# t-neumann/versalignLib

Hardware: AMD Instinct MI355X
Metric: GCUPS (giga DP cell updates/sec) SW affine-gap, 150x500 bp (higher is better)
Workload: dtype int16; 1 GPU; 1048576 pairs/GPU, 150 bp x 500 bp, SW affine-gap int16 score (open -5, extend -1), inputs resident in HBM; pairs_per_gpu=1048576, read_length=150, ref_length=500, kernel_geometry=16x10

## Files before the change

### versalignlib_amd/csrc/cell_rules.h

```cpp
#pragma once

#include <algorithm>
#include <cstdlib>
#include <stdexcept>
#include <string>

#include "cell_constants.h"

namespace valign {

struct RuleInputs {
    Scoring sc;
    int R = 0, F = 0;
    bool sse_policy = false;
    bool no_sym = false, no_tag = false, no_f16 = false, no_prof_key = false;
    bool no_max3 = false;
    bool no_tilt = false;
};

inline long long nw_tilt_span(const Scoring &sc, int rows, int F) {
    const long long per_row = -(long long)(sc.affine ? sc.ext_ref : sc.gap_ref);
    const long long per_col = -(long long)(sc.affine ? sc.ext_read : sc.gap_read);
    return per_row * (rows + 1) + per_col * (F + 1);
}

inline bool half_float_exact(const Scoring &sc, int alg, int R, int F, int rows) {
    const long long top = (long long)std::min(R, F) * std::max({sc.match, sc.mismatch, 0});
    long long slack = std::max({std::abs(sc.match), std::abs(sc.mismatch), std::abs(sc.open_read),
                                std::abs(sc.ext_read), std::abs(sc.open_ref), std::abs(sc.ext_ref)});
    if (alg == kAlgSW) return top + 2 * slack <= 2048 && slack <= 1024;
    if (!sc.affine) slack = std::max<long long>(slack, std::max(std::abs(sc.gap_read), std::abs(sc.gap_ref)));
    const long long span = nw_tilt_span(sc, rows, F);
    const long long centre = (top + span) / 2;
    return span < 30000 && (top + span - centre) + 3 * slack <= 2048 && centre + 3 * slack <= 2048 && slack <= 512;
}

inline bool half_float_unit_exact(const Scoring &sc, int R, int F) {
    const long long top = (long long)std::min(R, F) * std::max({sc.match, sc.mismatch, 0});
    const long long slack = std::max({std::abs(sc.match), std::abs(sc.mismatch), std::abs(sc.gap_read), std::abs(sc.gap_ref)});
    return top + 2 * slack < 1024 && slack < 512;
// ... 89 lines not shown
    if (sc.open_ref > 0 || sc.ext_ref > 0) return false;
    const long long B = sym_affine_bias(sc);
    const long long hi = (long long)std::min(R, F) * std::max({sc.match, sc.mismatch, 0}) + 1;
    return B - kMax3WindowLow <= 1024 && B + hi <= kMax3WindowHigh;
}
inline const char *ran_sym_affine_name(bool max3) { return max3 ? "max3" : "sources"; }

inline int sym_affine_tilt_bias(const Scoring &sc) {
    const int o = -sc.open_ref, x = -sc.ext_ref, m = std::max({0, -sc.mismatch, -sc.match});
    return kMax3WindowLow + std::max(o - x, m);
}
inline long long sym_affine_tilt_top_index(int R, int F, int rows, int K) {
    const int lead = rows > R ? (rows - R) / K : 0;
    return (long long)rows + F - lead;
}
inline bool sym_affine_tilt_ok(const RuleInputs &in, int R, int F, int rows, int K) {
    if (in.no_tilt || K > kTiltMaxK || !sym_affine_max3_ok(in, R, F)) return false;
    const Scoring &sc = in.sc;
    const long long B = sym_affine_tilt_bias(sc);
    const long long hi = (long long)std::min(R, F) * std::max({sc.match, sc.mismatch, 0}) + 1;
    return B + (long long)-sc.ext_ref * sym_affine_tilt_top_index(R, F, rows, K) + hi <= kMax3WindowHigh;
}
inline const char *ran_sym_affine_frame_name(bool tilted) { return tilted ? "tilted" : "plain"; }

struct FillChoice {
    int kernel = 0;
    bool affine_tagged = false, tagged = false;
};
inline FillChoice fill_choice(const RuleInputs &in, int alg, int G, int K) {
    const Scoring &sc = in.sc;
    FillChoice c;
    const int rows = G * K;
    c.affine_tagged = sc.affine && !in.sse_policy && !in.no_tag && affine_tagged_range_ok(in, alg, rows, K);
    c.tagged = !sc.affine && !in.no_tag && tagged_range_ok(in, alg, rows);
    const bool lane_key = c.tagged && alg == kAlgSW && lane_key_ok(in, K);
    const bool prof_key = lane_key && prof_key_ok(in, K);
    const bool affine_sym = sc.affine && sc.open_read == sc.open_ref && sc.ext_read == sc.ext_ref && !in.no_sym;
    if (prof_key) c.kernel = kFillTagProfKey;
    else if (c.tagged) c.kernel = in.sse_policy ? (lane_key ? kFillSseTagKey : kFillSseTag) : (lane_key ? kFillTagKey : kFillTag);
    else if (in.sse_policy) c.kernel = kFillSse;
    else if (sc.affine) c.kernel = c.affine_tagged ? (affine_sym ? kFillAffineTagSym : kFillAffineTag) : (affine_sym ? kFillAffineSym : kFillAffine);
    else c.kernel = (sc.gap_read == sc.gap_ref && !in.no_sym) ? kFillLinearSym : kFillLinear;
    return c;
}

constexpr int placed_key_bits(int K) { return K <= 4 ? 2 : (K <= 8 ? 3 : 4); }
// ... 255 lines not shown
```

### versalignlib_amd/csrc/dp_kernels.hip.h

```cpp
#pragma once

#include <hip/hip_runtime.h>
#include <stdint.h>

#include <type_traits>
#include <utility>

#include "base_classes.h"
#include "cell_constants.h"

namespace valign {

typedef short s16x2 __attribute__((ext_vector_type(2)));
typedef _Float16 f16x2 __attribute__((ext_vector_type(2)));
typedef unsigned short u16x2 __attribute__((ext_vector_type(2)));

constexpr int kWave = 64;
constexpr int kWaveLanes = 64;
constexpr int kCodePad = 72;
constexpr short kNegInf = -16384;

constexpr int kMaxScoreGroups = 16;
constexpr int kOneSweep = 0x7FFFFFFF;

// ... 369 lines not shown
    }
    if (live) {
        for (int idx = lane; idx < geo::kPairStride / 4; idx += kWave) {
            const unsigned lo = (unsigned short)(zero_score + row_key_step * (15 - (2 * idx) % K) + ((2 * idx) % K == 0 ? row0_score : 0));
            const unsigned hi = (unsigned short)(zero_score + row_key_step * (15 - (2 * idx + 1) % K) + ((2 * idx + 1) % K == 0 ? row0_score : 0));
            reinterpret_cast<unsigned *>(prof + geo::kZeroSlab * geo::kPairStride)[idx] = lo | (hi << 16);
        }
    }
    __syncthreads();
#pragma unroll
    for (int d = kWave / 2; d >= 1; d >>= 1) {
        const int other = __shfl_xor(cols_used, d, kWave);
        cols_used = other > cols_used ? other : cols_used;
    }
    w.cols_used = __builtin_amdgcn_readfirstlane(cols_used);
    w.prof = prof;
    w.refc = refc + 2 * kCodePad;
    w.first_bad = first_bad;
    w.pair0 = pair0;
    w.last = last;
    return live;
}

template <int K>
__device__ __forceinline__ void lds_load_lane(unsigned addr, unsigned (&v)[K / 2]) {
    constexpr int N = K / 2;
    if constexpr ((K * 2) % 16 == 0) {
#pragma unroll
        for (int i = 0; i < N / 4; ++i) {
            const u32x4 x = *(lds_cu32x4 *)(addr + 16 * i);
            v[4 * i] = x.x; v[4 * i + 1] = x.y; v[4 * i + 2] = x.z; v[4 * i + 3] = x.w;
        }
    } else if constexpr ((K * 2) % 8 == 0) {
#pragma unroll
        for (int i = 0; i < N / 2; ++i) {
            const u32x2 x = *(lds_cu32x2 *)(addr + 8 * i);
            v[2 * i] = x.x; v[2 * i + 1] = x.y;
        }
    } else {
#pragma unroll
        for (int i = 0; i < N; ++i) v[i] = *(lds_cu32 *)(addr + 4 * i);
    }
}

template <int K>
__device__ __forceinline__ void merge_profile(const unsigned (&va)[K / 2], const unsigned (&vb)[K / 2], s16x2 (&S)[K]) {
// ... 62 lines not shown
    int fold = tilt_row + tilt_col;
    short s_row0 = 0;
    if constexpr (SOURCES && K <= kTiltMaxK) {
        if (args.sym_max3_bias > 0 && (args.sym_max3_bias >> 16) != 0) {
            fold = -2 * (int)args.ext_ref;
            s_row0 = (short)((int)args.ext_ref - (int)args.open_ref);
        }
    }
    const int centre = (HALF && TILT) ? nw_frame_centre(args.R, F_batch, G * K, args.match, args.mismatch, tilt_row, tilt_col) : 0;
    const int rcentre = (HALF && TILT) ? nw_frame_centre(args.R, F_batch, G * K, args.match, args.mismatch, 0, 0) : 0;
    const float unit = LINF16_SW ? 1.0f / 1024.0f : 1.0f;
    auto cell = [](int v) __attribute__((always_inline)) {
        return HALF ? pk(__builtin_bit_cast(short, (_Float16)v)) : pk((short)v);
    };
    auto cell_add = [](s16x2 a, s16x2 b) __attribute__((always_inline)) {
        return HALF ? __builtin_bit_cast(s16x2, __builtin_bit_cast(f16x2, a) + __builtin_bit_cast(f16x2, b)) : a + b;
    };
    auto cell_sub = [](s16x2 a, s16x2 b) __attribute__((always_inline)) {
        return HALF ? __builtin_bit_cast(s16x2, __builtin_bit_cast(f16x2, a) - __builtin_bit_cast(f16x2, b)) : a - b;
    };
    const short s_match = HALF ? __builtin_bit_cast(short, (_Float16)(((int)args.match + fold) * unit)) : (short)(args.match + fold);
    const short s_mismatch = HALF ? __builtin_bit_cast(short, (_Float16)(((int)args.mismatch + fold) * unit)) : (short)(args.mismatch + fold);
    const short s_zero = HALF ? __builtin_bit_cast(short, (_Float16)fold) : (short)fold;
    if (!wave_setup<G, K, false>(reads, refs, n_pairs, args.R, F_batch, args.prof_area, args.refc_stride,
                                 args.wave_lds, s_match, s_mismatch, w, false, block, s_zero, kOneSweep, 0, s_row0))
        return;
    const long long pair0 = w.pair0;
    const int F = (ALG == kAlgSW) ? w.cols_used : F_batch;

    const unsigned lmask = l == 0 ? 0u : 0xFFFFFFFFu;
    const unsigned lane_base = lds_offset(w.prof) + l * geo::kLaneBytes;
    const int lead = (ALG == kAlgSW && G * K > args.R) ? (G * K - args.R) / K : 0;
    unsigned code_addr = lds_offset(w.refc) + grp * args.refc_stride - 2 * (l - lead);

    s16x2 g_read, g_ref, o_read, e_read, o_ref, e_ref;
    if (ALG == kAlgSW) {
        g_read = pk((short)-args.gap_read);   g_ref = pk((short)-args.gap_ref);
        o_read = pk((short)-args.open_read);  e_read = pk((short)-args.ext_read);
        o_ref = pk((short)-args.open_ref);    e_ref = pk((short)-args.ext_ref);
    } else {
        g_read = g_ref = e_read = e_ref = pk(0);
        o_read = pk((short)(args.open_read - args.ext_read));
        o_ref = pk((short)(args.open_ref - args.ext_ref));
    }
    const s16x2 border_f = pk(ALG == kAlgNW ? (F16 ? (short)0xFC00 : kNegInf) : (short)0);
    const _Float16 open_h = (_Float16)(int)(TILT ? args.open_ref - args.ext_ref : args.open_ref), ext_h = (_Float16)(int)args.ext_ref;
    const _Float16 open_rd = (_Float16)(int)(TILT ? args.open_read - args.ext_read : args.open_read), ext_rd = (_Float16)(int)args.ext_read;
    const f16x2 o_half = f16x2{open_h, open_h}, e_half = f16x2{ext_h, ext_h}, zero_half = f16x2{(_Float16)0, (_Float16)0};
// ... 5 lines not shown
        Hl[q] = cell(tilt_row * (l * K + q) - centre);
        El[q] = border_f;
        HOl[q] = (ALG == kAlgSW) ? pk(0) : (F16 ? cell_add(Hl[q], pk(__builtin_bit_cast(short, open_h))) : Hl[q] + o_ref);
    }
    s16x2 up0 = pk(0), h_last = Hl[K - 1], f_last = border_f, best = pk(0);
    s16x2 fup_keep = border_f;
    s16x2 row_best = cell(-rcentre);
    int j = -l;
    s16x2 top_row = pk(0), top_step = pk(0), row_tilt = pk(0);
    const s16x2 col_step = cell(tilt_col);
    if (TILT) {
        if (l == 0) {
            top_row = cell(-tilt_row + tilt_col - centre);
            top_step = col_step;
            up0 = cell(-tilt_row - centre);
        }
        row_tilt = cell(tilt_row * (G * K - 1) + tilt_col * (1 - l) - centre + rcentre);
    }

    constexpr bool PIPE = true;
    unsigned pa[K / 2], pb[K / 2];
    s16x2 S0[K], S1[K];
    unsigned ca_next = 0, cb_next = 0;
    if (PIPE) {
        const unsigned ca = *(lds_cu8 *)(code_addr), cb = *(lds_cu8 *)(code_addr + 1);
        lds_load_lane<K>(lane_base + ca * geo::kPairStride, pa);
        lds_load_lane<K>(lane_base + cb * geo::kPairStride, pb);
        ca_next = *(lds_cu8 *)(code_addr + 2);
        cb_next = *(lds_cu8 *)(code_addr + 3);
    }

    lds_cu8 *code_ptr = (lds_cu8 *)code_addr;

    auto step = [&](auto masked_tag, auto track_tag, s16x2 (&S)[K], s16x2 (&Snext)[K]) __attribute__((always_inline)) {
        constexpr bool MASKED = decltype(masked_tag)::value;
        constexpr int TRACK = decltype(track_tag)::value;
        const s16x2 diag0 = up0;
        if (G == 16) {
            up0 = as_pk((unsigned)__builtin_amdgcn_update_dpp(0, (int)as_u32(h_last), 0x111, 0xF, 0xF, true));
        } else {
            up0 = as_pk(from_prev_lane(as_u32(h_last)) & lmask);
        }
        if (TILT) up0 = as_pk(as_u32(up0) | as_u32(top_row));
        s16x2 fup0 = border_f;
        if (AFFINE && !SOURCES) {
            if (G == 16 && ALG == kAlgSW) {
                fup0 = as_pk((unsigned)__builtin_amdgcn_update_dpp(0, (int)as_u32(f_last), 0x111, 0xF, 0xF, true));
// ... 210 lines not shown
        if constexpr (SOURCES) {
            biased = args.sym_max3_bias > 0;
            const bool tilted = K <= kTiltMaxK && biased && (args.sym_max3_bias >> 16) != 0;
            if constexpr (K <= kTiltMaxK) if (tilted) {
                const int B = args.sym_max3_bias & 0xFFFF, xi = -(int)args.ext_ref;
                const int oxi = -(int)args.open_ref - xi;
                const s16x2 ox_c = pk((short)oxi), kx_c = pk((short)(K * xi));
                const int u0 = l * (K - 1);
                s16x2 lead_border = as_pk(as_u32(pk((short)(B + xi - oxi))) & ~lmask);
                const s16x2 lead_step = as_pk(as_u32(pk((short)xi)) & ~lmask);
                const int s0 = K - steps % K;
                s16x2 fl[K], acc[K], dprev[K];
#pragma unroll
                for (int q = 0; q < K; ++q) {
                    Hl[q] = El[q] = pk((short)(B + xi * (u0 + q + 1)));
                    HOl[q] = Hl[q] - ox_c;
                    int c = q - s0;
                    c += c < 0 ? K : 0;
                    fl[q] = acc[q] = pk((short)(B + xi * (u0 + c + 2)));
                    dprev[q] = Hl[q];
                }
                up0 = pk((short)(B + xi * u0 - oxi));
                f_last = HOl[K - 1];
                auto tilted_step = [&](auto slot_tag) __attribute__((always_inline)) {
                    constexpr int SLOT0 = decltype(slot_tag)::value;
                    s16x2 S[K], d[K];
                    const s16x2 diag0 = up0;
                    up0 = group_prev_or<G>(HOl[K - 1], lead_border, lmask);
                    lead_border = lead_border + lead_step;
                    merge_profile<K>(pa, pb, S);
                    lds_load_lane<K>(lane_base + ca_next * geo::kPairStride, pa);
                    lds_load_lane<K>(lane_base + cb_next * geo::kPairStride, pb);
                    ca_next = ((volatile lds_cu8 *)code_ptr)[4];
                    cb_next = ((volatile lds_cu8 *)code_ptr)[5];
                    s16x2 e_cur;
                    auto pass1 = [&](int q, s16x2 &e) __attribute__((always_inline)) {
                        d[q] = (q == 0 ? diag0 : Hl[q - 1]) + S[q];
                        e = pk_max3_h(El[q], HOl[q], fl[(q + SLOT0) % K]);
                        El[q] = e;
                    };
                    s16x2 ho = up0;
                    pass1(0, e_cur);
                    s16x2 f = as_pk(group_prev_or_zero<G>(as_u32(f_last), lmask)), h = pk(0);
#pragma unroll
                    for (int q = 0; q < K; ++q) {
                        f = pk_max_h(f, ho);
                        s16x2 e_next = pk(0);
                        if (q + 1 < K) pass1(q + 1, e_next);
                        h = pk_max3_h(d[q], e_cur, f);
                        Hl[q] = h;
                        ho = h - ox_c;
                        HOl[q] = ho;
                        if (!(q & 1)) {
                            s16x2 &a = acc[(q + SLOT0) % K];
                            a = pk_max3_h(a, d[q], dprev[q + 1]);
                        }
                        e_cur = e_next;
                    }
#pragma unroll
                    for (int q = 1; q < K; q += 2) dprev[q] = d[q];
                    f_last = f;
                    acc[SLOT0 % K] = acc[SLOT0 % K] + kx_c;
                    fl[SLOT0 % K] = fl[SLOT0 % K] + kx_c;
                    code_ptr += 2;
                };
                unrolled_steps(std::make_integer_sequence<int, K>{}, [&](auto slot_tag) __attribute__((always_inline)) {
                    if constexpr (decltype(slot_tag)::value > 0) {
                        if (decltype(slot_tag)::value >= s0) tilted_step(slot_tag);
                    }
                });
                for (int trips = steps / K; trips > 0; --trips)
                    unrolled_steps(std::make_integer_sequence<int, K>{}, [&](auto slot_tag) __attribute__((always_inline)) { tilted_step(slot_tag); });
                best = pk(0);
#pragma unroll
                for (int q = 0; q < K; q += 2) acc[q] = pk_max_h(acc[q], dprev[q + 1]);
#pragma unroll
                for (int q = 0; q < K; ++q) best = pk_max(best, acc[q] - fl[q]);
            }
            if (biased && !tilted) {
                const s16x2 bias_c = pk((short)args.sym_max3_bias);
                const s16x2 lead_bias = as_pk(as_u32(bias_c) & ~lmask);
                auto biased_step = [&](s16x2 (&S)[K]) __attribute__((always_inline)) {
                    const s16x2 diag0 = up0;
                    up0 = group_prev_or<G>(h_last, lead_bias, lmask);
                    merge_profile<K>(pa, pb, S);
                    lds_load_lane<K>(lane_base + ca_next * geo::kPairStride, pa);
                    lds_load_lane<K>(lane_base + cb_next * geo::kPairStride, pb);
                    ca_next = code_ptr[4];
                    cb_next = code_ptr[5];
                    s16x2 d_cur, e_cur, d_prev = bias_c;
                    auto pass1 = [&](int q, s16x2 &d, s16x2 &e) __attribute__((always_inline)) {
                        d = (q == 0 ? diag0 : Hl[q - 1]) + S[q];
                        e = pk_max3_h(El[q] - e_read, HOl[q], bias_c);
                        El[q] = e;
                    };
// ... 90 lines not shown
        } else {
            if (pa < n_pairs) scores[pa] = res.x;
            if (pa + 1 < n_pairs) scores[pa + 1] = res.y;
        }
    }
}

struct WaveLds {
    int prof_area, refc_stride, total;
};

template <int G, int K>
inline WaveLds wave_lds(int R, int F) {
    using geo = Geo<G, K>;
    WaveLds w;
    const int raw_refs = ((2 * F + 16 + 15) / 16) * 16;
    w.prof_area = geo::kProfBytes > raw_refs ? geo::kProfBytes : raw_refs;
    w.prof_area = ((w.prof_area + 15) / 16) * 16;
    w.refc_stride = ((2 * (F + 2 * kCodePad) + 15) / 16) * 16;
    w.total = w.prof_area + geo::kGroups * w.refc_stride + ((geo::kPairs * 8 + 15) / 16) * 16;
    return w;
}

}
```

### versalignlib_amd/csrc/engine.hip.h

```cpp
#pragma once

#include <hip/hip_runtime.h>
#include <stdint.h>
#include <stdio.h>
#include <stdlib.h>
#include <string.h>

#include <algorithm>
#include <atomic>
#include <chrono>
#include <condition_variable>
#include <functional>
#include <map>
#include <memory>
#include <mutex>
#include <stdexcept>
#include <string>
#include <thread>
#include <utility>
#include <vector>

#include "align_parts.h"
#include "cell_rules.h"
#include "hip_handles.h"
// ... 92 lines not shown
};
constexpr int kNumGeometries = sizeof(kGeometries) / sizeof(kGeometries[0]);
#define VALIGN_COUNT(G, K) +1
static_assert(kNumGeometries == 0 VALIGN_ALL_PARTS(VALIGN_COUNT, VALIGN_COUNT), "kernel_instances.hip.h lists other geometries than this table");
#undef VALIGN_COUNT

constexpr int kMaxBlockLds = 160 * 1024;
constexpr int kSlots = 4;
constexpr int kDefaultBlockLds = 64 * 1024;

struct LaunchPlan {
    bool long_mode = false;
    const Geometry *geo = nullptr;
    WaveLds lds{};
    int waves_per_block = 4;
    int pairs_per_wave = 0;
};

class DebugSwitches {
public:
    DebugSwitches() {
        const char *env = getenv("VALIGN_HIP_DEBUG");
        if (!env) return;
        static const char *const known[] = {"no_sym", "no_tag", "no_f16", "no_max3", "no_tilt", "no_fused", "no_prof_key", "no_overlap", "no_band_chain",
                                            "force_long", "wide_align", "strip_k", "no_single_strip", "no_direct_out", "ragged_min", "chunk_bytes",
                                            "align_chunk_bytes", "direct_bytes", "scratch_cap_mb", "whole_rows", "short_strips", "cigar_rows_mb", "cigar_lanes",
                                            "span_scratch_bytes", "subopt_scratch_bytes", "span_cigar_mb"};
        std::string s(env);
        for (size_t at = 0; at <= s.size();) {
            const size_t end = std::min(s.find(',', at), s.size());
            const std::string item = s.substr(at, end - at);
            at = end + 1;
            if (item.empty()) continue;
            const size_t eq = item.find('=');
            const std::string name = item.substr(0, eq);
            bool ok = false;
            for (const char *k : known) ok = ok || name == k;
            if (!ok) throw std::runtime_error("VALIGN_HIP_DEBUG: unknown switch '" + name + "'");
            kv_[name] = eq == std::string::npos ? 1 : atoll(item.c_str() + eq + 1);
        }
    }
    bool on(const char *name) const { return kv_.count(name) != 0; }
    long long value(const char *name, long long fallback) const {
        auto it = kv_.find(name);
        return it == kv_.end() ? fallback : it->second;
    }

// ... 99 lines not shown
    void launch_score(const LaunchPlan &plan, int alg, int R, int F, long long n, const uint8_t *d_reads,
                      const uint8_t *d_refs, int16_t *d_scores, hipStream_t stream,
                      const LengthGroup *groups = nullptr, int n_groups = 0);


    void launch_unpack(const uint8_t *d_packed, uint8_t *d_out, long long n, int len, hipStream_t stream);

    LongFacts long_facts(int alg) const {
        return LongFacts{band_width_, band_nw_, score_wide_cells(alg), dbg_.on("short_strips"), dbg_.on("no_single_strip"), no_band_chain_, band_plan_.usable};
    }
    LongScoreMode long_mode(int alg, bool refuse) const { return long_score_mode(rule_inputs(), alg, long_facts(alg), refuse); }

    void score_long_device(int alg, long long n, const uint8_t *d_reads, const uint8_t *d_refs, int16_t *d_scores, hipStream_t stream);
    void sync_band_tables(hipStream_t stream);
    void score_band_device(const LongScoreMode &mode, long long n, const uint8_t *d_reads, const uint8_t *d_refs, int16_t *d_scores, PlacedRec *d_placed,
                           hipStream_t stream);

    const char *score_cell_format(int alg, long long n = 0) const;
    std::string ran_score_cells() const;
    const char *ran_align_fill() const { return ran_align_fill_; }
    static std::string ran_geometry(const Geometry *g) { return g ? std::to_string(g->G) + "x" + std::to_string(g->K) : "none"; }
    std::string ran_kernels() const;

    RuleInputs rule_inputs() const { return RuleInputs{sc_, R_, F_, sse_policy_, no_sym_, no_tag_, no_f16_, no_prof_key_, no_max3_, no_tilt_}; }
    bool score_int16_ok(int alg) const;
    bool score_wide_cells(int alg) const { return score_width_ == 32 || (score_width_ == 0 && !score_int16_ok(alg)); }

    void score_host(int opt, int n, const char *const *reads, const char *const *refs, short *scores,
                    int threads, int16_t *d_dest = nullptr);



    struct WalkChain {
        int region;
        long long chunk_pairs;
        int *min_start;
        uint8_t *packed;
    };
    hipEvent_t trace_done(int region) const { return trace_done_[region].get(); }
    const LaunchPlan &align_plan_for(int alg, FillChoice &choice);
    const LaunchPlan &align_base_plan() const {
        if (plan_.long_mode && align_resident_.geo && !align_resident_.long_mode && R_ <= 1024 && align_resident_.lds.total <= 140 * 1024) {
            const int wpb = align_resident_.waves_per_block;
            const int waves_per_cu = (kMaxBlockLds / std::max(1, align_resident_.lds.total * wpb)) * wpb;
            if (waves_per_cu >= 2 || !sc_.affine) return align_resident_;
        }
        return plan_;
// ... 294 lines not shown
    bool band_nw_ = false;
    bool band_placed_ = false;
    bool placed_wide_ = false;
    bool trace_checkpoints_ = false;
    int score_width_ = 0;
    int ragged_ = 0, force_g_ = 0, force_k_ = 0;
    size_t score_chunk_bytes_ = 48u << 20;
    size_t align_chunk_bytes_ = 128u << 20;
    size_t direct_bytes_ = 768u << 10;
    long long ragged_min_ = 2048;
    std::vector<int> read_caps_, ref_caps_;
    std::vector<unsigned char> read_class_;
    std::vector<unsigned short> ref_class_;
    std::map<std::pair<int, int>, LaunchPlan> class_plans_;
    hipStream_t ragged_dev_stream_ = nullptr;
    HostPacker packer_{R_, F_};
    HostStats host_stats_;
    DebugSwitches dbg_;
    bool no_sym_ = dbg_.on("no_sym");
    bool no_tag_ = dbg_.on("no_tag");
    bool no_f16_ = dbg_.on("no_f16");
    bool no_max3_ = dbg_.on("no_max3");
    bool no_tilt_ = dbg_.on("no_tilt");
    bool no_fused_ = dbg_.on("no_fused");
    bool no_prof_key_ = dbg_.on("no_prof_key");
    bool copy_engines_primed_ = false;
    std::unique_ptr<CopyIssuer> copy_issuer_;
    bool wide_align_ = dbg_.on("wide_align");
    bool whole_rows_ = dbg_.on("whole_rows");
    bool no_direct_out_ = dbg_.on("no_direct_out");
    bool no_overlap_ = dbg_.on("no_overlap");
    int strip_k_ = (int)dbg_.value("strip_k", 0);
    long long scratch_cap_mb_ = dbg_.value("scratch_cap_mb", 0);
    bool chain_regions_busy_[2] = {false, false};
    std::string arch_;
    LaunchPlan plan_, latency_plan_;
    LaunchPlan base_plan_;
    LaunchPlan align_resident_;
    LaunchPlan fallback_plan_;
    long long slot_begin_[kSlots] = {}, slot_pending_[kSlots] = {};
    long long staged_pairs_ = 0, align_staged_pairs_ = 0;
    size_t record_staged_bytes_ = 0;
    bool pack_ = true;
    BandPlan band_plan_;
    int band_tables_width_ = -1;
    int band_blocks_per_cu_ = 0, band_lds_ = 0;
    int long_strip_rows_ = 0;
    static constexpr unsigned kRanF16 = 1, kRanInt16 = 2, kRanInt32 = 4;
    unsigned ran_score_cells_ = 0;
    const char *ran_align_fill_ = "none";
    const Geometry *ran_score_geo_ = nullptr, *ran_align_geo_ = nullptr;
    const Geometry *ran_placed_geo_ = nullptr, *ran_subopt_geo_ = nullptr, *ran_extend_geo_ = nullptr;
    const char *ran_score_sym_affine_ = nullptr;
    const char *ran_score_sym_affine_frame_ = "plain";
    const char *ran_placed_ = "none";
    std::string ran_span_ = "none";
    size_t span_scratch_bytes_ = (size_t)dbg_.value("span_scratch_bytes", 256ll << 20);
    std::string ran_span_cigar_ = "none";
    size_t span_cigar_bytes_ = (size_t)std::max(0ll, dbg_.value("span_cigar_mb", 768)) << 20;
    const char *ran_subopt_ = "none";
    int subopt_ring_cols_ = 0;
    size_t subopt_scratch_bytes_ = (size_t)dbg_.value("subopt_scratch_bytes", 256ll << 20);
    const char *ran_extend_ = "none";
    const char *ran_result_format_ = "rows";
    long long cigar_d2h_bytes_ = 0;
    const CigarSink *cigar_ = nullptr;
    long long cigar_pairs_[2] = {0, 0};
    long long align_ptr_bytes_per_pair_ = 0;
    long long align_ckpt_bytes_per_pair_ = 0;
    int cu_count_ = 0;
    bool no_band_chain_ = dbg_.on("no_band_chain");
    int start_col_[kSlots] = {};

    StreamHandle streams_[kSlots];
    EventHandle slot_done_[kSlots];
    EventHandle in_done_[kSlots], kernels_done_[kSlots];
    StreamHandle trace_stream_;
// ... 43 lines not shown
```

### versalignlib_amd/csrc/engine_core.hip

```cpp
#include "engine.hip.h"

namespace valign {

Engine::Engine(int device, int R, int F, const Scoring &sc, int force_g, int force_k)
    : device_(device), R_(R), F_(F), sc_(sc) {
    if (R < 0 || F < 0) throw std::runtime_error("negative sequence length");
    if ((long long)R + F > 32767)
        throw std::runtime_error("read_length + ref_length exceeds the ABI's 16-bit coordinates");
    validate_scoring();
    int count = 0;
    hip_check(hipGetDeviceCount(&count), "hipGetDeviceCount");
    if (device < 0 || device >= count)
        throw std::runtime_error("HIP device " + std::to_string(device) + " not present (" +
                                 std::to_string(count) + " visible): libHIPKernel.so has no CPU path");
    hip_check(hipSetDevice(device_), "hipSetDevice");
    hipDeviceProp_t prop;
    hip_check(hipGetDeviceProperties(&prop, device_), "hipGetDeviceProperties");
    arch_ = prop.gcnArchName;
    cu_count_ = prop.multiProcessorCount;
    if (arch_.find("gfx950") == std::string::npos)
        throw std::runtime_error("device is " + arch_ + "; this library carries gfx950 code only");
    force_g_ = force_g;
    force_k_ = force_k;
    plan_ = choose_plan(R_, F_, force_g, force_k);
// ... 74 lines not shown
             "\"ran_span_cigar\": \"%s\", \"span_cigar_scratch_bytes\": %lld, "
             "\"ran_subopt\": \"%s\", \"subopt_scratch_bytes\": %lld, \"subopt_ring_cols\": %d, \"ran_extend\": \"%s\", "
             "\"ran_score_geometry\": \"%s\", \"ran_align_geometry\": \"%s\", "
             "\"ran_placed_geometry\": \"%s\", \"ran_subopt_geometry\": \"%s\", \"ran_extend_geometry\": \"%s\"}",
             arch_.c_str(), device_, opt & 0xF, sc_.affine ? 1 : 0, plan_.geo->G, plan_.geo->K,
             plan_.geo->G * plan_.geo->K, plan_.pairs_per_wave, plan_.waves_per_block, plan_.lds.total,
             plan_.lds.total * plan_.waves_per_block, F_ + plan_.geo->G - 1, n > 0 ? (n + ppb - 1) / ppb : 0,
             plan_.long_mode ? 1 : 0, band_width_, ragged_, host_stats_.launches,
             host_stats_.cells_padded > 0 ? host_stats_.cells_swept / host_stats_.cells_padded : 1.0,
             score_cell_format(opt & 0xF, n), host_stats_.direct, host_stats_.packed, host_stats_.direct_out,
             ((opt & 0xF) == kAlgSW || band_nw_) ? band_rows : VALIGN_HIP_BAND_BLOCK_ROWS, ((opt & 0xF) == kAlgSW || band_nw_) ? band_align : VALIGN_HIP_BAND_COL_ALIGN,
             band_blocks_per_cu_, band_lds_, (band_tables_width_ == band_width_ && band_plan_.usable) ? band_plan_.cells : 0ll, long_strip_rows_, host_stats_.d2h_row_bytes / 1e6, host_stats_.full_row_bytes / 1e6, host_stats_.gather_ms, host_stats_.classify_ms, host_stats_.wait_ms,
             host_stats_.drain_ms, ran_score_cells().c_str(), ran_align_fill_, band_alignments(), band_nw(), band_placed(), align_ptr_bytes_per_pair_, trace_checkpoints(),
             align_ckpt_bytes_per_pair_, (long long)d_ptr_.bytes(), ran_result_format_, cigar_d2h_bytes_,
             (long long)(d_cig_rows_[0].bytes() + d_cig_rows_[1].bytes()), ran_placed_, placed_wide(), (long long)(d_placed_rows_.bytes() + d_placed_ends_.bytes()),
             ran_span_.c_str(), span_ref_length(rule_inputs()), (long long)span_[kSlots].bytes(),
             ran_span_cigar_.c_str(), (long long)(span_cigar_[0].bytes() + span_cigar_[1].bytes()),
             ran_subopt_, (long long)subopt_[kSlots].bytes(), subopt_ring_cols_, ran_extend_,
             ran_geometry(ran_score_geo_).c_str(), ran_geometry(ran_align_geo_).c_str(),
             ran_geometry(ran_placed_geo_).c_str(), ran_geometry(ran_subopt_geo_).c_str(), ran_geometry(ran_extend_geo_).c_str());
    std::string out(buf);
    if (ran_score_sym_affine_)
        out.insert(out.size() - 1, std::string(", \"ran_score_sym_affine\": \"") + ran_score_sym_affine_ + "\", \"ran_score_sym_affine_frame\": \"" +
                                       ran_score_sym_affine_frame_ + "\"");
    return out;
}

void Engine::band_block_shape(int &block_rows, int &col_align) const {
    const bool chain = long_mode(kAlgSW, false).chain;
    block_rows = chain ? kBandK : VALIGN_HIP_BAND_BLOCK_ROWS;
    col_align = chain ? VALIGN_HIP_BAND_CHAIN_COL_ALIGN : VALIGN_HIP_BAND_COL_ALIGN;
}

void Engine::validate_scoring() {
    auto fits = [](int v) { return v >= -32768 && v <= 32767; };
    if (!fits(sc_.match) || !fits(sc_.mismatch) || !fits(sc_.gap_read) || !fits(sc_.gap_ref) ||
        !fits(sc_.open_read) || !fits(sc_.ext_read) || !fits(sc_.open_ref) || !fits(sc_.ext_ref))
        throw std::runtime_error("scoring parameter outside int16");
    const bool gaps_ok = sc_.affine ? (sc_.open_read <= 0 && sc_.ext_read <= 0 && sc_.open_ref <= 0 && sc_.ext_ref <= 0)
                                    : (sc_.gap_read <= 0 && sc_.gap_ref <= 0);
    if (!gaps_ok) throw std::runtime_error("positive gap scores are not supported by the HIP kernels");
    if (sc_.affine && (sc_.ext_read < sc_.open_read || sc_.ext_ref < sc_.open_ref))
        throw std::runtime_error("affine gap scores need extend >= open in each direction (an extension dearer "
                                 "than the opening is not an affine model)");
}

LaunchPlan Engine::choose_plan(int R, int F, int force_g, int force_k, bool latency, bool full_only) const {
// ... 166 lines not shown
```

### versalignlib_amd/csrc/engine_score.hip

```cpp
#define VALIGN_TU_SCORE 1
#include "engine.hip.h"

namespace valign {

void Engine::score_device(int opt, long long n, const uint8_t *d_reads, const uint8_t *d_refs,
                  int16_t *d_scores, hipStream_t stream, bool length_sorted) {
    const int alg = opt & 0xF;
    if (alg > 1 || n <= 0) return;
    hip_check(hipSetDevice(device_), "hipSetDevice");
    if (length_sorted) {
        host_stats_ = HostStats{};
        ran_score_cells_ = 0;
        ran_score_geo_ = nullptr;
        ran_score_sym_affine_ = nullptr;
    }
    if (score_width_ == 16 && !score_int16_ok(alg))
        throw std::runtime_error("shape x scoring can leave the int16 range of the DP cells (read_length " +
                                 std::to_string(R_) + ", ref_length " + std::to_string(F_) + ")");
    const bool wide = score_wide_cells(alg);
    if (plan_.long_mode || wide) {
        score_long_device(alg, n, d_reads, d_refs, d_scores, stream);
        return;
    }
    if (length_sorted && ragged_applies(alg) && ragged_fits(n) && n >= 2 * ragged_min_) {
// ... 30 lines not shown
            blocks += (groups[g].pairs + pairs_per_block - 1) / pairs_per_block;
            if (blocks > 0x7FFFFFFFll) throw std::runtime_error("batch too large for one launch");
            a.groups[g].block_end = (unsigned)blocks;
            a.groups[g].F = groups[g].F;
            a.groups[g].n = groups[g].pairs;
            a.groups[g].pair_ofs = groups[g].pair_ofs;
            a.groups[g].read_ofs = (long long)groups[g].read_ofs;
            a.groups[g].ref_ofs = (long long)groups[g].ref_ofs;
        }
    }
    a.prof_area = plan.lds.prof_area;
    a.refc_stride = plan.lds.refc_stride;
    a.wave_lds = plan.lds.total;
    put_scoring(a);
    const int gaps = score_gap_form(rule_inputs(), alg, R, F, plan.geo->G * plan.geo->K);
    const void *fn = plan.geo->kernel[alg][gaps];
    ran_score_cells_ |= gap_form_f16(gaps) ? kRanF16 : kRanInt16;
    ran_score_geo_ = plan.geo;
    if (alg == kAlgSW && gaps == kGapAffineSym) {
        const bool max3 = sym_affine_max3_ok(rule_inputs(), R_, F_);
        a.sym_max3_bias = max3 ? sym_affine_bias(sc_) : 0;
        const bool tilted = sym_affine_tilt_ok(rule_inputs(), R_, F_, plan.geo->G * plan.geo->K, plan.geo->K);
        if (tilted) a.sym_max3_bias = sym_affine_tilt_bias(sc_) | 1 << 16;
        ran_score_sym_affine_ = ran_sym_affine_name(max3);
        ran_score_sym_affine_frame_ = ran_sym_affine_frame_name(tilted);
    }
    const int block_lds = plan.lds.total * plan.waves_per_block;
    if (block_lds > kDefaultBlockLds)
        hip_check(hipFuncSetAttribute(fn, hipFuncAttributeMaxDynamicSharedMemorySize, block_lds),
                  "hipFuncSetAttribute(MaxDynamicSharedMemorySize)");
    if (blocks > 0x7FFFFFFFll) throw std::runtime_error("batch too large for one launch");
    if (blocks == 0) return;
    void *kargs[] = {&a};
    hip_check(hipLaunchKernel(fn, dim3((unsigned)blocks), dim3(plan.waves_per_block * kWave), kargs,
                              (size_t)block_lds, stream),
              "hipLaunchKernel(score_kernel)");
}

void Engine::launch_unpack(const uint8_t *d_packed, uint8_t *d_out, long long n, int len, hipStream_t stream) {
    if (n <= 0 || len <= 0) return;
    UnpackArgs a{d_packed, d_out, n, len};
    void *kargs[] = {&a};
    const bool even = (len & 1) == 0;
    const long long items = even ? (n * (long long)(len / 2) + 7) / 8 : n * (long long)((len + 1) / 2);
    const long long blocks = (items + 255) / 256;
    if (blocks > 0x7FFFFFFFll) throw std::runtime_error("batch too large for one launch");
    hip_check(hipLaunchKernel(even ? (const void *)&unpack_even_kernel : (const void *)&unpack_odd_kernel, dim3((unsigned)blocks),
                              dim3(256), kargs, 0, stream),
              "hipLaunchKernel(unpack_kernel)");
}
// ... 348 lines not shown
```

Baseline: 8964 GCUPS.

## Use per-lane register score tables with byte-select streams in tilted affine SW

Adds a row-table path for the tilted symmetric-affine SW kernel. Each lane builds packed byte tables of substitution scores for its read rows in registers, and the reference is rewritten as per-column perm selectors in LDS. Each DP step then fetches one selector dword and uses v_perm to form the scores, instead of loading profile rows from LDS indexed by reference codes. This lowers LDS traffic per step and shrinks the LDS footprint, but adds register pressure (Ta/Tb arrays), a more complex setup phase and an extra repair variant for non-ACGT columns.

After: 9607 GCUPS (median of 6 runs). 7.2% higher.

```diff
diff --git a/versalignlib_amd/csrc/cell_rules.h b/versalignlib_amd/csrc/cell_rules.h
--- a/versalignlib_amd/csrc/cell_rules.h
+++ b/versalignlib_amd/csrc/cell_rules.h
@@ -16,6 +16,7 @@
     bool no_sym = false, no_tag = false, no_f16 = false, no_prof_key = false;
     bool no_max3 = false;
     bool no_tilt = false;
+    bool no_row_tables = false;
 };
 
 inline long long nw_tilt_span(const Scoring &sc, int rows, int F) {
@@ -151,6 +152,17 @@
     return B + (long long)-sc.ext_ref * sym_affine_tilt_top_index(R, F, rows, K) + hi <= kMax3WindowHigh;
 }
 inline const char *ran_sym_affine_frame_name(bool tilted) { return tilted ? "tilted" : "plain"; }
+
+inline int sym_affine_row_table_low(const Scoring &sc) { return std::min({sc.match, sc.mismatch, 0}) - 2 * sc.ext_ref; }
+inline int sym_affine_row_table_high(const Scoring &sc) {
+    return std::max({sc.match, sc.mismatch, 0}) - 2 * sc.ext_ref + (sc.ext_ref - sc.open_ref);
+}
+inline bool sym_affine_row_tables_ok(const RuleInputs &in, int R, int F, int rows, int K, int lds_profile, int lds_tables) {
+    if (in.no_row_tables || !sym_affine_tilt_ok(in, R, F, rows, K)) return false;
+    if (in.sc.ext_ref - in.sc.open_ref < 0 || F > 60000) return false;
+    return sym_affine_row_table_low(in.sc) >= 0 && sym_affine_row_table_high(in.sc) <= 255 && lds_tables <= lds_profile;
+}
+inline const char *ran_sym_affine_scores_name(bool row_tables) { return row_tables ? "row_tables" : "lds_profile"; }
 
 struct FillChoice {
     int kernel = 0;
diff --git a/versalignlib_amd/csrc/dp_kernels.hip.h b/versalignlib_amd/csrc/dp_kernels.hip.h
--- a/versalignlib_amd/csrc/dp_kernels.hip.h
+++ b/versalignlib_amd/csrc/dp_kernels.hip.h
@@ -415,6 +415,146 @@
     return live;
 }
 
+constexpr int row_table_pad(int G) { return G + 4; }
+constexpr unsigned kSelZero4 = 0x0c0c0c0cu;
+
+template <int G, int K>
+__device__ __forceinline__ bool wave_setup_tables(const uint8_t *reads, const uint8_t *refs, long long n, int R, int F,
+                                                  int refs_area, int sel_stride, int wave_lds, short match, short mismatch,
+                                                  short zero_score, short row0_score, unsigned block, WaveTables &w,
+                                                  unsigned (&Ta)[K], unsigned (&Tb)[K], bool &repair) {
+    using geo = Geo<G, K>;
+    constexpr int kPad = row_table_pad(G);
+    const int lane = threadIdx.x & (kWave - 1);
+    const int wave = threadIdx.x / kWave;
+    const int row0 = R - geo::kRows;
+
+    unsigned char *raw = valign_smem + (size_t)wave * wave_lds;
+    unsigned char *sel = raw + refs_area;
+
+    const int waves = blockDim.x / kWave;
+    const long long pair0 = ((long long)block * waves + wave) * geo::kPairs;
+    const bool live = pair0 < n;
+    long long pair_end = pair0 + geo::kPairs;
+    if (pair_end > n) pair_end = n;
+    const int last = (int)(pair_end - pair0) - 1;
+
+    if (live) {
+        stage_span(raw, refs, pair0 * F, pair_end * F, lane);
+        stage_span(sel, reads, pair0 * R, pair_end * R, lane);
+    }
+    __syncthreads();
+
+    if (live) {
+        auto table = [&](int c, unsigned &lo, unsigned &hi) __attribute__((always_inline)) {
+            unsigned b[8];
+#pragma unroll
+            for (int a = 0; a < 8; ++a) b[a] = (unsigned)(a >= 1 && a <= 4 ? (a == c + 1 ? match : mismatch) : zero_score) & 0xFFu;
+            lo = b[0] | b[1] << 8 | b[2] << 16 | b[3] << 24;
+            hi = b[4] | b[5] << 8 | b[6] << 16 | b[7] << 24;
+        };
+        unsigned t_lo[4], t_hi[4];
+#pragma unroll
+        for (int c = 0; c < 4; ++c) table(c, t_lo[c], t_hi[c]);
+        const unsigned char *raw_rd = sel + (int)((unsigned long long)(reads + pair0 * R) & 15ull);
+        const int grp = lane / G, l = lane % G;
+#pragma unroll
+        for (int half = 0; half < 2; ++half) {
+            int p = 2 * grp + half;
+            p = p > last ? last : p;
+#pragma unroll
+            for (int q0 = 0; q0 < K; q0 += 4) {
+                const int pos = row0 + l * K + q0;
+                const int at = pos < -3 ? -3 : pos;
+                unsigned w4 = lds_dword_at(raw_rd + p * R + at);
+                if (pos < 0) w4 = pos < -3 ? 0u : w4 & (0xFFFFFFFFu << (8 * -pos));
+                const unsigned cls = base_class4(w4);
+                unsigned col[4];
+#pragma unroll
+                for (int c = 0; c < 4; ++c) col[c] = select_bytes8(t_hi[c], t_lo[c], cls);
+                const unsigned lo01 = __builtin_amdgcn_perm(col[1], col[0], 0x05010400u), hi01 = __builtin_amdgcn_perm(col[1], col[0], 0x07030602u);
+                const unsigned lo23 = __builtin_amdgcn_perm(col[3], col[2], 0x05010400u), hi23 = __builtin_amdgcn_perm(col[3], col[2], 0x07030602u);
+                unsigned (&T)[K] = half ? Tb : Ta;
+                T[q0] = __builtin_amdgcn_perm(lo23, lo01, 0x05040100u);
+                T[q0 + 1] = __builtin_amdgcn_perm(lo23, lo01, 0x07060302u);
+                if (q0 + 2 < K) {
+                    T[q0 + 2] = __builtin_amdgcn_perm(hi23, hi01, 0x05040100u);
+                    T[q0 + 3] = __builtin_amdgcn_perm(hi23, hi01, 0x07060302u);
+                }
+            }
+        }
+        const unsigned r4 = ((unsigned)row0_score & 0xFFu) * 0x01010101u;
+        Ta[0] += r4;
+        Tb[0] += r4;
+    }
+    __syncthreads();
+
+    int cols_used = 0;
+    bool before_last = false;
+    unsigned *stream = reinterpret_cast<unsigned *>(sel);
+    const int stride_dw = sel_stride / 4;
+    if (live) {
+        for (int idx = lane; idx < geo::kGroups * 2 * kPad; idx += kWave) {
+            const int g = idx / (2 * kPad), x = idx - g * (2 * kPad);
+            stream[g * stride_dw + (x < kPad ? x : F + x)] = kSelZero4;
+        }
+        const int ref_skew = (int)((unsigned long long)(refs + pair0 * F) & 15ull);
+        typedef unsigned short u16;
+#pragma unroll
+        for (int g = 0; g < geo::kGroups; ++g) {
+            int pa = 2 * g, pb = 2 * g + 1;
+            pa = pa > last ? last : pa;
+            pb = pb > last ? last : pb;
+            const unsigned char *raw_a = raw + ref_skew + pa * F, *raw_b = raw + ref_skew + pb * F;
+            unsigned *out_g = stream + g * stride_dw + kPad;
+            u16x2 ends_a = u16x2{0, 0}, ends_b = u16x2{0, 0};
+            auto note = [](u16x2 &ends, unsigned acgt, int j) __attribute__((always_inline)) {
+                const unsigned none = ~nonzero_bytes(acgt) & 0x80808080u;
+                const u16 end = acgt ? (u16)(j + 4 - (__builtin_clz(acgt) >> 3)) : (u16)0;
+                const u16 first_none = none ? (u16)(0xFFFF - (j + (__builtin_ctz(none) >> 3))) : (u16)0;
+                ends = __builtin_elementwise_max(ends, u16x2{end, first_none});
+            };
+            const int F4 = F & ~3;
+            for (int j = 4 * lane; j < F4; j += 4 * kWave) {
+                const unsigned ca = base_class4(lds_dword_at(raw_a + j)), cb = base_class4(lds_dword_at(raw_b + j));
+                const unsigned sa = select_bytes8(0x0c0c0c03u, 0x0201000cu, ca), sb = select_bytes8(0x0c0c0c07u, 0x0605040cu, cb);
+                uint4 s;
+                s.x = __builtin_amdgcn_perm(sb, sa, 0x0c040c00u) | 0x0c000c00u;
+                s.y = __builtin_amdgcn_perm(sb, sa, 0x0c050c01u) | 0x0c000c00u;
+                s.z = __builtin_amdgcn_perm(sb, sa, 0x0c060c02u) | 0x0c000c00u;
+                s.w = __builtin_amdgcn_perm(sb, sa, 0x0c070c03u) | 0x0c000c00u;
+                *reinterpret_cast<uint4 *>(out_g + j) = s;
+                note(ends_a, sa ^ kSelZero4, j);
+                note(ends_b, sb ^ kSelZero4, j);
+            }
+            for (int j = F4 + lane; j < F; j += kWave) {
+                const int ca = base_class(raw_a[j]), cb = base_class(raw_b[j]);
+                const bool va = ca >= 1 && ca <= 4, vb = cb >= 1 && cb <= 4;
+                out_g[j] = (va ? (unsigned)(ca - 1) : 0x0cu) | (vb ? (unsigned)(cb + 3) : 0x0cu) << 16 | 0x0c000c00u;
+                ends_a = __builtin_elementwise_max(ends_a, u16x2{va ? (u16)(j + 1) : (u16)0, va ? (u16)0 : (u16)(0xFFFF - j)});
+                ends_b = __builtin_elementwise_max(ends_b, u16x2{vb ? (u16)(j + 1) : (u16)0, vb ? (u16)0 : (u16)(0xFFFF - j)});
+            }
+#pragma unroll
+            for (int d = kWave / 2; d >= 1; d >>= 1) {
+                ends_a = __builtin_elementwise_max(ends_a, __builtin_bit_cast(u16x2, __shfl_xor(__builtin_bit_cast(int, ends_a), d, kWave)));
+                ends_b = __builtin_elementwise_max(ends_b, __builtin_bit_cast(u16x2, __shfl_xor(__builtin_bit_cast(int, ends_b), d, kWave)));
+            }
+            before_last |= 0xFFFF - (int)ends_a.y < (int)ends_a.x || 0xFFFF - (int)ends_b.y < (int)ends_b.x;
+            cols_used = (int)ends_a.x > cols_used ? (int)ends_a.x : cols_used;
+            cols_used = (int)ends_b.x > cols_used ? (int)ends_b.x : cols_used;
+        }
+    }
+    __syncthreads();
+    repair = __builtin_amdgcn_readfirstlane((int)before_last) != 0;
+    w.cols_used = __builtin_amdgcn_readfirstlane(cols_used);
+    w.prof = raw;
+    w.refc = reinterpret_cast<unsigned char *>(stream + kPad);
+    w.first_bad = nullptr;
+    w.pair0 = pair0;
+    w.last = last;
+    return live;
+}
+
 template <int K>
 __device__ __forceinline__ void lds_load_lane(unsigned addr, unsigned (&v)[K / 2]) {
     constexpr int N = K / 2;
@@ -523,8 +663,20 @@
     const short s_match = HALF ? __builtin_bit_cast(short, (_Float16)(((int)args.match + fold) * unit)) : (short)(args.match + fold);
     const short s_mismatch = HALF ? __builtin_bit_cast(short, (_Float16)(((int)args.mismatch + fold) * unit)) : (short)(args.mismatch + fold);
     const short s_zero = HALF ? __builtin_bit_cast(short, (_Float16)fold) : (short)fold;
-    if (!wave_setup<G, K, false>(reads, refs, n_pairs, args.R, F_batch, args.prof_area, args.refc_stride,
-                                 args.wave_lds, s_match, s_mismatch, w, false, block, s_zero, kOneSweep, 0, s_row0))
+    bool tables = false, repair = false;
+    unsigned Ta[K], Tb[K];
+    if constexpr (SOURCES && K <= kTiltMaxK) {
+        tables = args.sym_max3_bias > 0 && (args.sym_max3_bias >> 16 & 3) == 3;
+        bool live = false;
+        if (tables)
+            live = wave_setup_tables<G, K>(reads, refs, n_pairs, args.R, F_batch, args.prof_area, args.refc_stride, args.wave_lds,
+                                           s_match, s_mismatch, s_zero, s_row0, block, w, Ta, Tb, repair);
+        if (!tables)
+            live = wave_setup<G, K, false>(reads, refs, n_pairs, args.R, F_batch, args.prof_area, args.refc_stride,
+                                           args.wave_lds, s_match, s_mismatch, w, false, block, s_zero, kOneSweep, 0, s_row0);
+        if (!live) return;
+    } else if (!wave_setup<G, K, false>(reads, refs, n_pairs, args.R, F_batch, args.prof_area, args.refc_stride,
+                                        args.wave_lds, s_match, s_mismatch, w, false, block, s_zero, kOneSweep, 0, s_row0))
         return;
     const long long pair0 = w.pair0;
     const int F = (ALG == kAlgSW) ? w.cols_used : F_batch;
@@ -576,7 +728,7 @@
     unsigned pa[K / 2], pb[K / 2];
     s16x2 S0[K], S1[K];
     unsigned ca_next = 0, cb_next = 0;
-    if (PIPE) {
+    if (PIPE && !tables) {
         const unsigned ca = *(lds_cu8 *)(code_addr), cb = *(lds_cu8 *)(code_addr + 1);
         lds_load_lane<K>(lane_base + ca * geo::kPairStride, pa);
         lds_load_lane<K>(lane_base + cb * geo::kPairStride, pb);
@@ -833,17 +985,40 @@
                 }
                 up0 = pk((short)(B + xi * u0 - oxi));
                 f_last = HOl[K - 1];
-                auto tilted_step = [&](auto slot_tag) __attribute__((always_inline)) {
+                constexpr int kLdsProfile = 0, kRowTables = 1, kRowTablesRepair = 2;
+                lds_cu32 *sel_ptr = (lds_cu32 *)(lds_offset(w.refc) + grp * args.refc_stride - 4 * (l - lead));
+                unsigned sel_cur = 0, sel_next = 0;
+                if (tables) {
+                    sel_cur = sel_ptr[0];
+                    sel_next = sel_ptr[1];
+                }
+                const unsigned zero_q = as_u32(pk(s_zero)), zero_0 = as_u32(pk((short)(s_zero + s_row0)));
+                auto tilted_step = [&](auto slot_tag, auto form_tag) __attribute__((always_inline)) {
                     constexpr int SLOT0 = decltype(slot_tag)::value;
+                    constexpr int FORM = decltype(form_tag)::value;
                     s16x2 S[K], d[K];
                     const s16x2 diag0 = up0;
                     up0 = group_prev_or<G>(HOl[K - 1], lead_border, lmask);
                     lead_border = lead_border + lead_step;
-                    merge_profile<K>(pa, pb, S);
-                    lds_load_lane<K>(lane_base + ca_next * geo::kPairStride, pa);
-                    lds_load_lane<K>(lane_base + cb_next * geo::kPairStride, pb);
-                    ca_next = ((volatile lds_cu8 *)code_ptr)[4];
-                    cb_next = ((volatile lds_cu8 *)code_ptr)[5];
+                    if constexpr (FORM == kLdsProfile) {
+                        merge_profile<K>(pa, pb, S);
+                        lds_load_lane<K>(lane_base + ca_next * geo::kPairStride, pa);
+                        lds_load_lane<K>(lane_base + cb_next * geo::kPairStride, pb);
+                        ca_next = ((volatile lds_cu8 *)code_ptr)[4];
+                        cb_next = ((volatile lds_cu8 *)code_ptr)[5];
+                    } else {
+#pragma unroll
+                        for (int q = 0; q < K; ++q) S[q] = as_pk(__builtin_amdgcn_perm(Tb[q], Ta[q], sel_cur));
+                        if constexpr (FORM == kRowTablesRepair) {
+                            const unsigned none = ((sel_cur >> 3) & 0x00010001u) * 0xFFFFu;
+                            const unsigned fix_0 = zero_0 & none, fix_q = zero_q & none;
+#pragma unroll
+                            for (int q = 0; q < K; ++q) S[q] = as_pk(as_u32(S[q]) | (q == 0 ? fix_0 : fix_q));
+                        }
+                        sel_cur = sel_next;
+                        sel_next = ((volatile lds_cu32 *)sel_ptr)[2];
+                        sel_ptr += 1;
+                    }
                     s16x2 e_cur;
                     auto pass1 = [&](int q, s16x2 &e) __attribute__((always_inline)) {
                         d[q] = (q == 0 ? diag0 : Hl[q - 1]) + S[q];
@@ -873,15 +1048,23 @@
                     f_last = f;
                     acc[SLOT0 % K] = acc[SLOT0 % K] + kx_c;
                     fl[SLOT0 % K] = fl[SLOT0 % K] + kx_c;
-                    code_ptr += 2;
+                    if constexpr (FORM == kLdsProfile) code_ptr += 2;
                 };
-                unrolled_steps(std::make_integer_sequence<int, K>{}, [&](auto slot_tag) __attribute__((always_inline)) {
-                    if constexpr (decltype(slot_tag)::value > 0) {
-                        if (decltype(slot_tag)::value >= s0) tilted_step(slot_tag);
-                    }
-                });
-                for (int trips = steps / K; trips > 0; --trips)
-                    unrolled_steps(std::make_integer_sequence<int, K>{}, [&](auto slot_tag) __attribute__((always_inline)) { tilted_step(slot_tag); });
+                auto tilted_sweep = [&](auto form_tag) __attribute__((always_inline)) {
+                    unrolled_steps(std::make_integer_sequence<int, K>{}, [&](auto slot_tag) __attribute__((always_inline)) {
+                        if constexpr (decltype(slot_tag)::value > 0) {
+                            if (decltype(slot_tag)::value >= s0) tilted_step(slot_tag, form_tag);
+                        }
+                    });
+                    for (int trips = steps / K; trips > 0; --trips)
+                        unrolled_steps(std::make_integer_sequence<int, K>{}, [&](auto slot_tag) __attribute__((always_inline)) { tilted_step(slot_tag, form_tag); });
+                };
+                int form = __builtin_amdgcn_readfirstlane(tables ? (repair ? kRowTablesRepair : kRowTables) : kLdsProfile);
+                if (form == kLdsProfile) tilted_sweep(std::integral_constant<int, kLdsProfile>{});
+                asm volatile("" : "+s"(form));
+                if (form == kRowTables) tilted_sweep(std::integral_constant<int, kRowTables>{});
+                asm volatile("" : "+s"(form));
+                if (form == kRowTablesRepair) tilted_sweep(std::integral_constant<int, kRowTablesRepair>{});
                 best = pk(0);
 #pragma unroll
                 for (int q = 0; q < K; q += 2) acc[q] = pk_max_h(acc[q], dprev[q + 1]);
@@ -1018,4 +1201,16 @@
     return w;
 }
 
-}
+inline WaveLds row_table_lds(int G, int R, int F) {
+    const int groups = kWave / G, pairs = 2 * groups;
+    WaveLds w;
+    w.prof_area = ((pairs * F + 32 + 15) / 16) * 16;
+    int stride_dw = F + 2 * row_table_pad(G);
+    stride_dw += ((G - stride_dw) % 64 + 64) % 64;
+    w.refc_stride = 4 * stride_dw;
+    const int streams = groups * w.refc_stride, raw_reads = ((pairs * R + 32 + 15) / 16) * 16;
+    w.total = w.prof_area + (streams > raw_reads ? streams : raw_reads);
+    return w;
+}
+
+}
diff --git a/versalignlib_amd/csrc/engine.hip.h b/versalignlib_amd/csrc/engine.hip.h
--- a/versalignlib_amd/csrc/engine.hip.h
+++ b/versalignlib_amd/csrc/engine.hip.h
@@ -138,7 +138,7 @@
     DebugSwitches() {
         const char *env = getenv("VALIGN_HIP_DEBUG");
         if (!env) return;
-        static const char *const known[] = {"no_sym", "no_tag", "no_f16", "no_max3", "no_tilt", "no_fused", "no_prof_key", "no_overlap", "no_band_chain",
+        static const char *const known[] = {"no_sym", "no_tag", "no_f16", "no_max3", "no_tilt", "no_row_tables", "no_fused", "no_prof_key", "no_overlap", "no_band_chain",
                                             "force_long", "wide_align", "strip_k", "no_single_strip", "no_direct_out", "ragged_min", "chunk_bytes",
                                             "align_chunk_bytes", "direct_bytes", "scratch_cap_mb", "whole_rows", "short_strips", "cigar_rows_mb", "cigar_lanes",
                                             "span_scratch_bytes", "subopt_scratch_bytes", "span_cigar_mb"};
@@ -284,7 +284,11 @@
     static std::string ran_geometry(const Geometry *g) { return g ? std::to_string(g->G) + "x" + std::to_string(g->K) : "none"; }
     std::string ran_kernels() const;
 
-    RuleInputs rule_inputs() const { return RuleInputs{sc_, R_, F_, sse_policy_, no_sym_, no_tag_, no_f16_, no_prof_key_, no_max3_, no_tilt_}; }
+    RuleInputs rule_inputs() const {
+        RuleInputs in = RuleInputs{sc_, R_, F_, sse_policy_, no_sym_, no_tag_, no_f16_, no_prof_key_, no_max3_, no_tilt_};
+        in.no_row_tables = no_row_tables_;
+        return in;
+    }
     bool score_int16_ok(int alg) const;
     bool score_wide_cells(int alg) const { return score_width_ == 32 || (score_width_ == 0 && !score_int16_ok(alg)); }
 
@@ -625,6 +629,7 @@
     bool no_f16_ = dbg_.on("no_f16");
     bool no_max3_ = dbg_.on("no_max3");
     bool no_tilt_ = dbg_.on("no_tilt");
+    bool no_row_tables_ = dbg_.on("no_row_tables");
     bool no_fused_ = dbg_.on("no_fused");
     bool no_prof_key_ = dbg_.on("no_prof_key");
     bool copy_engines_primed_ = false;
@@ -656,6 +661,7 @@
     const Geometry *ran_placed_geo_ = nullptr, *ran_subopt_geo_ = nullptr, *ran_extend_geo_ = nullptr;
     const char *ran_score_sym_affine_ = nullptr;
     const char *ran_score_sym_affine_frame_ = "plain";
+    const char *ran_score_sym_affine_scores_ = "lds_profile";
     const char *ran_placed_ = "none";
     std::string ran_span_ = "none";
     size_t span_scratch_bytes_ = (size_t)dbg_.value("span_scratch_bytes", 256ll << 20);
diff --git a/versalignlib_amd/csrc/engine_core.hip b/versalignlib_amd/csrc/engine_core.hip
--- a/versalignlib_amd/csrc/engine_core.hip
+++ b/versalignlib_amd/csrc/engine_core.hip
@@ -120,7 +120,7 @@
     std::string out(buf);
     if (ran_score_sym_affine_)
         out.insert(out.size() - 1, std::string(", \"ran_score_sym_affine\": \"") + ran_score_sym_affine_ + "\", \"ran_score_sym_affine_frame\": \"" +
-                                       ran_score_sym_affine_frame_ + "\"");
+                                       ran_score_sym_affine_frame_ + "\", \"ran_score_sym_affine_scores\": \"" + ran_score_sym_affine_scores_ + "\"");
     return out;
 }
 
diff --git a/versalignlib_amd/csrc/engine_score.hip b/versalignlib_amd/csrc/engine_score.hip
--- a/versalignlib_amd/csrc/engine_score.hip
+++ b/versalignlib_amd/csrc/engine_score.hip
@@ -76,10 +76,19 @@
         a.sym_max3_bias = max3 ? sym_affine_bias(sc_) : 0;
         const bool tilted = sym_affine_tilt_ok(rule_inputs(), R_, F_, plan.geo->G * plan.geo->K, plan.geo->K);
         if (tilted) a.sym_max3_bias = sym_affine_tilt_bias(sc_) | 1 << 16;
+        const WaveLds tables_lds = row_table_lds(plan.geo->G, R, F);
+        const bool row_tables = tilted && sym_affine_row_tables_ok(rule_inputs(), R_, F_, plan.geo->G * plan.geo->K, plan.geo->K, plan.lds.total, tables_lds.total);
+        if (row_tables) {
+            a.sym_max3_bias |= 1 << 17;
+            a.prof_area = tables_lds.prof_area;
+            a.refc_stride = tables_lds.refc_stride;
+            a.wave_lds = tables_lds.total;
+        }
         ran_score_sym_affine_ = ran_sym_affine_name(max3);
         ran_score_sym_affine_frame_ = ran_sym_affine_frame_name(tilted);
-    }
-    const int block_lds = plan.lds.total * plan.waves_per_block;
+        ran_score_sym_affine_scores_ = ran_sym_affine_scores_name(row_tables);
+    }
+    const int block_lds = a.wave_lds * plan.waves_per_block;
     if (block_lds > kDefaultBlockLds)
         hip_check(hipFuncSetAttribute(fn, hipFuncAttributeMaxDynamicSharedMemorySize, block_lds),
                   "hipFuncSetAttribute(MaxDynamicSharedMemorySize)");
```
